# esrice/trio_binning

Hardware: AMD Instinct MI355X
Metric: Gbases/sec classified (k=21, 2x300M k-mer tables) (higher is better)
Workload: dtype u64

## Files before the change

trio_binning_amd/csrc/tbk_count.cpp:

```cpp
#include <hip/hip_runtime.h>

#include <algorithm>
#include <atomic>
#include <cerrno>
#include <cstdarg>
#include <cstdio>
#include <cstdlib>
#include <cstring>
#include <fcntl.h>
#include <string>
#include <thread>
#include <unistd.h>
#include <vector>

#include "../../include/tbk.h"
#include "tbk_common.h"
#include "tbk_compact_host.h"

extern "C" void tbk_set_error_(int code, const char *msg);
extern "C" hipError_t tbk_launch_separate(const uint8_t *, const uint64_t *, uint64_t, uint8_t *, hipStream_t);
extern "C" hipError_t tbk_launch_count(const uint8_t *, uint64_t, uint64_t, uint64_t, int, uint64_t *, uint32_t, TbkMz, int *, unsigned long long *,
                                       hipStream_t);
extern "C" uint64_t tbk_probe_passes(uint64_t total);
extern "C" hipError_t tbk_launch_count_clamp(uint64_t *, uint32_t, TbkMz, hipStream_t);
extern "C" hipError_t tbk_launch_count_rehash(uint64_t *, uint32_t, TbkMz, uint64_t *, uint32_t, TbkMz, int *, hipStream_t);
extern "C" hipError_t tbk_launch_count_histogram(uint64_t *, uint32_t, TbkMz, unsigned long long *, hipStream_t);
extern "C" hipError_t tbk_launch_count_unique(uint64_t *, uint32_t, TbkMz, uint64_t *, uint32_t, TbkMz, int, uint32_t, uint32_t,
                                              uint64_t *, uint64_t, unsigned long long *, hipStream_t);
extern "C" hipError_t tbk_launch_sort_u64(const uint64_t *, uint64_t *, uint64_t, int, hipStream_t);
extern "C" hipError_t tbk_launch_retain(const uint8_t *, uint64_t, uint64_t *, uint64_t, hipStream_t);
extern "C" hipError_t tbk_launch_count_class(const uint64_t *, uint64_t, uint64_t, uint64_t, int, uint64_t *, uint32_t, TbkMz, int *, unsigned long long *,
                                             uint32_t, uint32_t, hipStream_t);
extern "C" hipError_t tbk_launch_count_distil(uint64_t *, uint32_t, TbkMz, uint32_t, uint64_t *, uint8_t *, uint64_t, unsigned long long *, hipStream_t);
extern "C" hipError_t tbk_launch_db_solid_keys(const uint64_t *, const uint8_t *, uint64_t, uint64_t *, uint64_t, unsigned long long *, hipStream_t);
extern "C" hipError_t tbk_launch_db_unique(const uint64_t *, const uint8_t *, uint64_t, const uint64_t *, uint64_t, int, uint32_t, uint32_t, uint64_t *,
                                           uint64_t, unsigned long long *, hipStream_t);

static int cfail(int code, const char *fmt, ...) {
    char buf[512];
    va_list ap;
    va_start(ap, fmt);
    vsnprintf(buf, sizeof buf, fmt, ap);
    va_end(ap);
    tbk_set_error_(code, buf);
    return code;
}
#define CHIP(expr)                                                                                                      \
    do {                                                                                                                \
        hipError_t e_ = (expr);                                                                                         \
        if (e_ != hipSuccess)                                                                                           \
            return cfail(e_ == hipErrorOutOfMemory ? TBK_ERR_NOMEM : TBK_ERR_HIP, "%s: %s", #expr, hipGetErrorString(e_)); \
    } while (0)

struct tbk_counter {
    int device = 0, k = 0;
    uint64_t *d_lines = nullptr;
    uint32_t n_buckets = 0;
    TbkMz mz{0, 0, 0, 0};
    int *d_failed = nullptr;
    unsigned long long *d_used = nullptr;
    uint64_t since_clamp = 0;
    uint64_t used = 0;
    double load = 0.6;
    uint8_t *d_raw = nullptr, *d_sep = nullptr;
    uint64_t *d_off = nullptr;
    size_t cap_raw = 0, cap_sep = 0, cap_reads = 0;
    uint64_t bases_added = 0, reads_added = 0;
    hipEvent_t ev0 = nullptr, ev1 = nullptr;
    uint64_t timed_launches = 0, timed_windows = 0;
    double timed_ms = 0.0;
    uint64_t peak_table_bytes = 0;
    bool finished = false;
    bool broken = false;
    int passes = 1;
    uint64_t store_limit = 0;
    struct Segment { uint64_t *d = nullptr; uint64_t cap = 0, used = 0; };
    struct Piece { uint32_t segment; uint64_t first, words; };
    std::vector<Segment> segments;
    std::vector<Piece> pieces;
    uint64_t store_bytes = 0, store_words = 0;
    struct ClassDb { uint64_t *d_keys = nullptr; uint8_t *d_counts = nullptr; uint64_t n = 0; };
    std::vector<ClassDb> db;
    uint64_t database_bytes = 0;
    unsigned long long *d_hist = nullptr;
    uint64_t hist[256] = {0};
    uint64_t distinct_done = 0;
    bool compress = false;
    tbk_hpc *hpc = nullptr;
    bool keep_singletons = false;
    uint32_t floor() const { return keep_singletons ? 1u : 2u; }
};

static int counter_device(const tbk_counter *c) {
    int n = 0;
    if (hipGetDeviceCount(&n) != hipSuccess || n <= 0) return cfail(TBK_ERR_NO_DEVICE, "no HIP device visible; libtbk_hip has no CPU fallback");
    CHIP(hipSetDevice(c->device));
    return TBK_OK;
}

static int alloc_lines(int k, uint64_t capacity, double load, uint64_t **d_lines, uint32_t *n_buckets, TbkMz *mz, uint64_t *peak) {
    uint64_t nb = (uint64_t)((double)capacity / (TBK_SLOTS_PER_BUCKET * load)) + 16;
    if (nb > 0x7FFFFFF0ull) return cfail(TBK_ERR_NOMEM, "%llu distinct k-mers are more than one table holds", (unsigned long long)capacity);
    const size_t bytes = (size_t)nb * 128;
    hipError_t e = hipMalloc((void **)d_lines, bytes);
    if (e == hipSuccess) e = hipMemset2D(*d_lines, 128, 0xFF, 64, nb);
    if (e == hipSuccess) e = hipMemset2D((uint8_t *)*d_lines + 64, 128, 0, 64, nb);
    if (e != hipSuccess) {
        if (*d_lines) (void)hipFree(*d_lines);
        *d_lines = nullptr;
        (void)hipGetLastError();
        return cfail(e == hipErrorOutOfMemory ? TBK_ERR_NOMEM : TBK_ERR_HIP, "counting table for %llu k-mers (%zu bytes): %s",
                     (unsigned long long)capacity, bytes, hipGetErrorString(e));
    }
    *n_buckets = (uint32_t)nb;
    if (peak && bytes > *peak) *peak = bytes;
    const char *ew = getenv("TBK_COUNT_W"), *em = getenv("TBK_COUNT_M");
    *mz = tbk_mz_params(k, ew ? atoi(ew) : 6, capacity, em ? atoi(em) : 0, 0);
    return TBK_OK;
}
// ... 31 lines not shown
    c->device = device; c->k = k;
    c->passes = o.passes; c->store_limit = o.store_limit_bytes;
    c->compress = o.compress != 0;
    c->keep_singletons = o.keep_singletons != 0;
    if (c->compress) {
        const int made = tbk_hpc_create(device, &c->hpc);
        if (made) { delete c; return made; }
    }
    if (c->passes > 1) capacity_kmers = std::max<uint64_t>(1, capacity_kmers / (uint64_t)c->passes);
    const char *ev = getenv("TBK_COUNT_LOAD");
    c->load = ev ? atof(ev) : 0.6;
    if (c->load < 0.05) c->load = 0.05;
    if (c->load > 0.9) c->load = 0.9;
    rc = alloc_lines(k, capacity_kmers, c->load, &c->d_lines, &c->n_buckets, &c->mz, &c->peak_table_bytes);
    hipError_t e = hipSuccess;
    if (!rc && c->passes > 1) {
        e = hipMalloc((void **)&c->d_hist, 256 * sizeof(unsigned long long));
        if (e == hipSuccess) e = hipMemset(c->d_hist, 0, 256 * sizeof(unsigned long long));
    }
    if (!rc) e = hipMalloc((void **)&c->d_failed, sizeof(int));
    if (!rc && e == hipSuccess) e = hipMalloc((void **)&c->d_used, 1025 * sizeof(unsigned long long));
    if (!rc && e == hipSuccess) e = hipMemset(c->d_failed, 0, sizeof(int));
    if (!rc && e == hipSuccess) e = hipMemset(c->d_used, 0, 1025 * sizeof(unsigned long long));
    if (!rc && e != hipSuccess) rc = cfail(TBK_ERR_HIP, "tbk_counter_create: %s", hipGetErrorString(e));
    if (rc) { tbk_counter_destroy(c); return rc; }
    *out = c;
    return TBK_OK;
}

static int counter_grow(tbk_counter *c, uint64_t capacity) {
    uint64_t *d_new = nullptr;
    uint32_t nb = 0;
    TbkMz mz{0, 0, 0, 0};
    int rc = alloc_lines(c->k, capacity, c->load, &d_new, &nb, &mz, &c->peak_table_bytes);
    if (rc) return rc;
    hipError_t e = tbk_launch_count_rehash(c->d_lines, c->n_buckets, c->mz, d_new, nb, mz, c->d_failed, nullptr);
    int failed = 0;
    if (e == hipSuccess) e = hipMemcpy(&failed, c->d_failed, sizeof failed, hipMemcpyDeviceToHost);
    if (e != hipSuccess || failed) {
        (void)hipFree(d_new);
        return cfail(TBK_ERR_HIP, "counting table rebuild failed: %s", e != hipSuccess ? hipGetErrorString(e) : "new table full");
    }
    (void)hipFree(c->d_lines);
    c->d_lines = d_new; c->n_buckets = nb; c->mz = mz;
    return TBK_OK;
}

extern "C" void tbk_counter_destroy(tbk_counter *c) {
    if (!c) return;
    if (hipSetDevice(c->device) == hipSuccess) {
        (void)hipDeviceSynchronize();
        if (c->ev0) (void)hipEventDestroy(c->ev0);
        if (c->ev1) (void)hipEventDestroy(c->ev1);
        for (void *p : {(void *)c->d_lines, (void *)c->d_failed, (void *)c->d_used, (void *)c->d_raw, (void *)c->d_sep, (void *)c->d_off, (void *)c->d_hist})
            if (p) (void)hipFree(p);
        for (const tbk_counter::Segment &s : c->segments)
            if (s.d) (void)hipFree(s.d);
        for (const tbk_counter::ClassDb &d : c->db) {
            if (d.d_keys) (void)hipFree(d.d_keys);
            if (d.d_counts) (void)hipFree(d.d_counts);
        }
    }
    tbk_hpc_destroy(c->hpc);
    delete c;
}

static int count_stream(tbk_counter *c, const void *d_stream, uint64_t sep_total, int cls) {
    const uint64_t passes = tbk_probe_passes(sep_total);
    for (uint64_t p0 = 0; p0 < passes;) {
        uint64_t slots = (uint64_t)c->n_buckets * TBK_SLOTS_PER_BUCKET;
        constexpr uint64_t piece_cap = 1u << 19;
        static_assert(piece_cap <= TBK_COUNT_GRID_BLOCKS, "a piece of count_stream must fit the grid of one tbk_count_kernel launch");
        const uint64_t piece = std::min<uint64_t>(std::max<uint64_t>(32768, slots / 4 / 2048), piece_cap);
        const uint64_t np = std::min(piece, passes - p0), windows = np * 2048;
        if ((double)(c->used + windows) > 0.85 * (double)slots) {
            uint64_t want = (uint64_t)((double)slots * c->load) * 2;
            while ((double)(c->used + windows) > 0.85 * ((double)want / c->load)) want *= 2;
            const int rc = counter_grow(c, want);
            if (rc) return rc;
            slots = (uint64_t)c->n_buckets * TBK_SLOTS_PER_BUCKET;
        }
        if (c->since_clamp + windows >= ((uint64_t)1 << 31)) {
            CHIP(tbk_launch_count_clamp(c->d_lines, c->n_buckets, c->mz, nullptr));
            c->since_clamp = 0;
        }
        c->since_clamp += windows;
        if (!c->ev0) { CHIP(hipEventCreate(&c->ev0)); CHIP(hipEventCreate(&c->ev1)); }
        CHIP(hipEventRecord(c->ev0, nullptr));
        if (cls < 0)
            CHIP(tbk_launch_count((const uint8_t *)d_stream, sep_total, p0, np, c->k, c->d_lines, c->n_buckets, c->mz, c->d_failed, c->d_used, nullptr));
        else
            CHIP(tbk_launch_count_class((const uint64_t *)d_stream, sep_total / 16, p0, np, c->k, c->d_lines, c->n_buckets, c->mz, c->d_failed, c->d_used,
                                        (uint32_t)c->passes, (uint32_t)cls, nullptr));
        CHIP(hipEventRecord(c->ev1, nullptr));
        int failed = 0;
        unsigned long long used = 0;
        CHIP(hipMemcpy(&failed, c->d_failed, sizeof failed, hipMemcpyDeviceToHost));
        {
            float ms = 0;
            CHIP(hipEventElapsedTime(&ms, c->ev0, c->ev1));
            c->timed_ms += ms; c->timed_launches++; c->timed_windows += std::min<uint64_t>(windows, sep_total - p0 * 2048);
        }
        CHIP(hipMemcpy(&used, c->d_used, sizeof used, hipMemcpyDeviceToHost));
        c->used = used;
        if (failed) return cfail(TBK_ERR_NOMEM, "counting table is full (%llu slots, %llu taken)", (unsigned long long)slots, used);
        p0 += np;
    }
    return TBK_OK;
}

static int store_append(tbk_counter *c, uint64_t sep_total, uint64_t **d_words, uint64_t *n_words) {
    const uint64_t words = (sep_total + 15) / 16;
    if (c->store_limit && (c->store_words + words) * 8 > c->store_limit)
        return cfail(TBK_ERR_NOMEM, "the retained store would pass its limit of %llu bytes: %llu bases are retained in %llu bytes, the next batch needs %llu more",
                     (unsigned long long)c->store_limit, (unsigned long long)c->bases_added, (unsigned long long)(c->store_words * 8),
                     (unsigned long long)(words * 8));
    if (c->segments.empty() || c->segments.back().cap - c->segments.back().used < words) {
        uint64_t cap = std::max<uint64_t>(words, std::max<uint64_t>((uint64_t)1 << 17, c->store_words / 2));
        if (c->store_limit) cap = std::max<uint64_t>(words, std::min<uint64_t>(cap, c->store_limit / 8 - c->store_words));
        tbk_counter::Segment seg;
        const hipError_t e = hipMalloc((void **)&seg.d, cap * 8);
        if (e != hipSuccess) {
            (void)hipGetLastError();
            return cfail(e == hipErrorOutOfMemory ? TBK_ERR_NOMEM : TBK_ERR_HIP, "the retained store cannot grow by %llu bytes (%s): %llu bases are retained in %llu bytes",
                         (unsigned long long)(cap * 8), hipGetErrorString(e), (unsigned long long)c->bases_added, (unsigned long long)c->store_bytes);
        }
        seg.cap = cap;
        c->segments.push_back(seg);
        c->store_bytes += cap * 8;
    }
    tbk_counter::Segment &seg = c->segments.back();
    CHIP(tbk_launch_retain(c->d_sep, sep_total, seg.d + seg.used, words, nullptr));
    c->pieces.push_back({(uint32_t)(c->segments.size() - 1), seg.used, words});
    *d_words = seg.d + seg.used;
    *n_words = words;
    seg.used += words;
    c->store_words += words;
    return TBK_OK;
}

static int distil_class(tbk_counter *c) {
    CHIP(tbk_launch_count_histogram(c->d_lines, c->n_buckets, c->mz, c->d_hist, nullptr));
    unsigned long long h[256];
    CHIP(hipMemcpy(h, c->d_hist, sizeof h, hipMemcpyDeviceToHost));
    uint64_t keep = 0;
    for (int i = (int)c->floor(); i < 256; i++) keep += h[i] - c->hist[i];
    c->distinct_done += h[0] - c->hist[0];
    for (int i = 0; i < 256; i++) c->hist[i] = h[i];
    tbk_counter::ClassDb d;
    c->db.push_back(d);
    tbk_counter::ClassDb &db = c->db.back();
    if (keep) {
        CHIP(hipMalloc((void **)&db.d_keys, keep * sizeof(uint64_t)));
        CHIP(hipMalloc((void **)&db.d_counts, keep));
    }
    unsigned long long got = 0;
    CHIP(hipMemset(c->d_used, 0, sizeof got));
    CHIP(tbk_launch_count_distil(c->d_lines, c->n_buckets, c->mz, c->floor(), db.d_keys, db.d_counts, keep, c->d_used, nullptr));
    CHIP(hipMemcpy(&got, c->d_used, sizeof got, hipMemcpyDeviceToHost));
    CHIP(hipMemset(c->d_used, 0, sizeof got));
    if (got != keep) return cfail(TBK_ERR_HIP, "distilling a class: %llu k-mers to keep by the histogram, %llu in the table", (unsigned long long)keep, got);
    db.n = keep;
    c->database_bytes += keep * 9;
    c->used = 0;
    c->since_clamp = 0;
    return TBK_OK;
}

static int counter_finish(tbk_counter *c) {
    if (c->finished) return TBK_OK;
    if (c->broken) return cfail(TBK_ERR_INVALID, "the counter failed while it was being finished");
    if (c->passes == 1) { c->finished = true; return TBK_OK; }
    int rc = counter_device(c);
    if (rc) return rc;
    c->broken = true;
    rc = distil_class(c);
    for (int cls = 1; !rc && cls < c->passes; cls++) {
        for (size_t i = 0; !rc && i < c->pieces.size(); i++) {
            const tbk_counter::Piece &pc = c->pieces[i];
            rc = count_stream(c, c->segments[pc.segment].d + pc.first, pc.words * 16, cls);
        }
        if (!rc) rc = distil_class(c);
    }
    if (rc) return rc;
    for (tbk_counter::Segment &sg : c->segments) (void)hipFree(sg.d);
    c->segments.clear(); c->pieces.clear();
    c->store_bytes = 0; c->store_words = 0;
    for (void **p : {(void **)&c->d_lines, (void **)&c->d_raw, (void **)&c->d_sep, (void **)&c->d_off}) {
        if (*p) (void)hipFree(*p);
        *p = nullptr;
    }
    c->n_buckets = 0; c->cap_raw = 0; c->cap_sep = 0; c->cap_reads = 0;
    tbk_hpc_destroy(c->hpc);
    c->hpc = nullptr;
    c->broken = false;
    c->finished = true;
    return TBK_OK;
}

extern "C" int tbk_counter_finish(tbk_counter *c) {
    if (!c) return cfail(TBK_ERR_INVALID, "counter is NULL");
    return counter_finish(c);
}

static int counter_run(tbk_counter *c, const uint8_t *d_bases, const uint64_t *d_offsets, uint64_t n_reads, uint64_t total) {
    if (c->hpc) {
        void *d_cb = nullptr, *d_co = nullptr;
        const int rc = tbk_hpc_compress_device(c->hpc, d_bases, d_offsets, n_reads, total, 1, &d_cb, &d_co, &total);
        if (rc) return rc;
        d_bases = (const uint8_t *)d_cb;
        d_offsets = (const uint64_t *)d_co;
    }
    const size_t need_sep = (size_t)total + n_reads + 64;
    if (need_sep > c->cap_sep) {
        if (c->d_sep) CHIP(hipFree(c->d_sep));
        c->d_sep = nullptr; c->cap_sep = 0;
        CHIP(hipMalloc((void **)&c->d_sep, need_sep + need_sep / 8));
        c->cap_sep = need_sep + need_sep / 8;
    }
    CHIP(tbk_launch_separate(d_bases, d_offsets, n_reads, c->d_sep, nullptr));
    const uint64_t sep_total = total + n_reads;
    int rc;
    if (c->passes > 1) {
        uint64_t *d_words = nullptr, n_words = 0;
        rc = store_append(c, sep_total, &d_words, &n_words);
        if (!rc) rc = count_stream(c, d_words, n_words * 16, 0);
    } else {
        rc = count_stream(c, c->d_sep, sep_total, -1);
    }
    if (rc) return rc;
    c->bases_added += total;
    c->reads_added += n_reads;
    return TBK_OK;
}

extern "C" int tbk_check_offsets_(const uint64_t *offsets, uint64_t n_reads);

extern "C" int tbk_counter_add_batch(tbk_counter *c, const uint8_t *bases, const uint64_t *offsets, uint64_t n_reads) {
    if (!c || (n_reads && (!bases || !offsets))) return cfail(TBK_ERR_INVALID, "NULL argument");
    if (c->finished || c->broken) return cfail(TBK_ERR_INVALID, "the counter is finished: no more reads can be added");
    if (!n_reads) return TBK_OK;
    int rc = tbk_check_offsets_(offsets, n_reads);
    if (rc) return rc;
    rc = counter_device(c);
    if (rc) return rc;
    const uint64_t total = offsets[n_reads];
    if (total + 16 > c->cap_raw) {
        if (c->d_raw) CHIP(hipFree(c->d_raw));
        c->d_raw = nullptr; c->cap_raw = 0;
        CHIP(hipMalloc((void **)&c->d_raw, total + total / 8 + 64));
        c->cap_raw = total + total / 8 + 64;
    }
    if (n_reads + 1 > c->cap_reads) {
        if (c->d_off) CHIP(hipFree(c->d_off));
        c->d_off = nullptr; c->cap_reads = 0;
        CHIP(hipMalloc((void **)&c->d_off, (n_reads + n_reads / 8 + 2) * sizeof(uint64_t)));
        c->cap_reads = n_reads + n_reads / 8 + 2;
    }
    CHIP(hipMemcpy(c->d_raw, bases, total, hipMemcpyHostToDevice));
    CHIP(hipMemcpy(c->d_off, offsets, (n_reads + 1) * sizeof(uint64_t), hipMemcpyHostToDevice));
    return counter_run(c, c->d_raw, c->d_off, n_reads, total);
}

extern "C" int tbk_counter_add_device(tbk_counter *c, const void *d_bases, const void *d_offsets, uint64_t n_reads, uint64_t total_bases) {
    if (!c || (n_reads && (!d_bases || !d_offsets))) return cfail(TBK_ERR_INVALID, "NULL argument");
    if (c->finished || c->broken) return cfail(TBK_ERR_INVALID, "the counter is finished: no more reads can be added");
    if (!n_reads) return TBK_OK;
    int rc = counter_device(c);
    if (rc) return rc;
    return counter_run(c, (const uint8_t *)d_bases, (const uint64_t *)d_offsets, n_reads, total_bases);
}

extern "C" int tbk_counter_kernel_timing(tbk_counter *c, uint64_t *launches, uint64_t *window_starts, double *total_ms, int reset) {
    if (!c) return cfail(TBK_ERR_INVALID, "counter is NULL");
    if (launches) *launches = c->timed_launches;
    if (window_starts) *window_starts = c->timed_windows;
    if (total_ms) *total_ms = c->timed_ms;
    if (reset) { c->timed_launches = 0; c->timed_windows = 0; c->timed_ms = 0.0; }
    return TBK_OK;
}

// ... 1104 lines not shown
```

trio_binning_amd/csrc/tbk_count_kernels.hip:

```cpp
#include <hip/hip_runtime.h>
#include <rocprim/device/device_scan.hpp>
#include <stdint.h>

#include <type_traits>

#include "tbk_common.h"
#include "tbk_compact.h"
#include "tbk_device.h"


static uint32_t g_stream_blocks = 0, g_entry_blocks = 0;
extern "C" int tbk_count_set_grid_caps_(uint32_t stream_blocks, uint32_t entry_blocks) {
    g_stream_blocks = stream_blocks;
    g_entry_blocks = entry_blocks;
    return 0;
}
static inline unsigned stream_grid(uint64_t blocks) { return (unsigned)(g_stream_blocks && blocks > g_stream_blocks ? g_stream_blocks : blocks); }
static inline unsigned entry_grid(uint64_t blocks) { return (unsigned)(g_entry_blocks && blocks > g_entry_blocks ? g_entry_blocks : blocks); }

__global__ void __launch_bounds__(256)
tbk_separate_kernel(const uint8_t *__restrict__ bases, const uint64_t *__restrict__ offsets, uint64_t n_reads,
                    uint8_t *__restrict__ out) {
    const uint32_t lane = threadIdx.x & 63u;
    const uint64_t waves = (uint64_t)gridDim.x * (blockDim.x >> 6);
    for (uint64_t r = (uint64_t)blockIdx.x * (blockDim.x >> 6) + (threadIdx.x >> 6); r < n_reads; r += waves) {
        const uint64_t lo = offsets[r], hi = offsets[r + 1];
        uint8_t *dst = out + lo + r;
        for (uint64_t i = lo + lane; i < hi; i += 64) dst[i - lo] = bases[i] & 0xDFu;
        if (lane == 0) dst[hi - lo] = 'N';
    }
}

__global__ void __launch_bounds__(256)
tbk_retain_kernel(const uint8_t *__restrict__ sep, uint64_t total, uint64_t *__restrict__ store, uint64_t n_chunks) {
    for (uint64_t c = (uint64_t)blockIdx.x * blockDim.x + threadIdx.x; c < n_chunks; c += (uint64_t)gridDim.x * blockDim.x)
        store[c] = load_chunk(sep, c * 16, total);
}

struct TbkClassSel {
    uint32_t n_classes, cls;
};

constexpr int TBK_COUNT_LINE = 16;
struct TbkCountView {
    uint64_t *lines;
    uint32_t n_buckets;
    TbkMz mz;
    __device__ __forceinline__ unsigned long long *keys(uint32_t b) const { return (unsigned long long *)(lines + (uint64_t)b * TBK_COUNT_LINE); }
    __device__ __forceinline__ uint32_t *counts(uint32_t b) const { return (uint32_t *)(lines + (uint64_t)b * TBK_COUNT_LINE + TBK_SLOTS_PER_BUCKET); }
};

constexpr uint32_t TBK_COUNT_MAX_WALK = 1u << 12;

__device__ __forceinline__ bool count_from(const TbkCountView &t, uint64_t key, uint32_t b, bool at_home, uint32_t n, uint32_t &claimed) {
    for (uint32_t walked = 0; walked <= t.n_buckets && walked < TBK_COUNT_MAX_WALK; walked++) {
        unsigned long long *line = t.keys(b);
        for (int s = 0; s < TBK_SLOTS_PER_BUCKET; s++) {
            unsigned long long cur = __hip_atomic_load(&line[s], __ATOMIC_RELAXED, __HIP_MEMORY_SCOPE_AGENT);
            if (cur == TBK_EMPTY) {
                cur = atomicCAS(&line[s], (unsigned long long)TBK_EMPTY, (unsigned long long)key);
                if (cur == TBK_EMPTY) { cur = key; claimed++; }
            }
            if (cur == key) { atomicAdd(&t.counts(b)[s], n); return true; }
        }
        b = tbk_next_bucket(key, t.mz, t.n_buckets, b, at_home && walked == 0);
    }
    return false;
}

template <int W, bool M64, typename... Sel>
__global__ void __launch_bounds__(64)
tbk_count_kernel(const uint8_t *__restrict__ bases, uint64_t total, uint64_t first_pass, uint64_t n_passes, int k, TbkCountView t,
                 int *__restrict__ failed, unsigned long long *__restrict__ used, Sel... sel) {
    static_assert(sizeof...(Sel) == 0 || (sizeof...(Sel) == 1 && (std::is_same<Sel, TbkClassSel>::value && ...)), "at most one class selector");
    constexpr bool PACKED = sizeof...(Sel) == 1;
    __shared__ uint64_t stage[TBK_CHUNKS + 2];
    const uint32_t lane = threadIdx.x & 63u;
    const uint64_t kmask = k == 32 ? ~0ull : ((1ull << (2 * k)) - 1ull);
    const uint32_t badk = k == 32 ? 0xFFFFFFFFu : ((1u << k) - 1u);
    using win_t = typename std::conditional<M64, uint64_t, uint32_t>::type;
    const int m = t.mz.m, o = t.mz.o;
    const uint64_t mmask = m >= 32 ? ~0ull : ((1ull << (2 * m)) - 1ull);
    auto mmer_order = [&](uint64_t fwd64, uint64_t rc64, uint32_t fsh, uint32_t bsh) -> win_t {
        if (M64) {
            const uint64_t x = (fwd64 >> fsh) & mmask, y = (rc64 >> bsh) & mmask;
            return (win_t)tbk_mmer_hash64(x < y ? x : y);
        }
        const uint32_t x = (uint32_t)(fwd64 >> fsh) & (uint32_t)mmask, y = (uint32_t)(rc64 >> bsh) & (uint32_t)mmask;
        return (win_t)tbk_mmer_hash(x < y ? x : y);
    };
    for (uint64_t pass = first_pass + blockIdx.x; pass < first_pass + n_passes; pass += gridDim.x) {
        const uint64_t P0 = pass * TBK_PASS;
        __builtin_amdgcn_fence(__ATOMIC_ACQ_REL, "wavefront");
        if constexpr (PACKED) {
            const uint64_t *store = reinterpret_cast<const uint64_t *>(bases);
            const uint64_t c0 = P0 / 16, n_chunks = total / 16;
            auto word = [&](uint64_t c) -> uint64_t { return c < n_chunks ? store[c] : 0xFFFFull << 32; };
            stage[lane] = word(c0 + lane);
            stage[64 + lane] = word(c0 + 64 + lane);
            if (lane < 2) stage[128 + lane] = word(c0 + 128 + lane);
        } else {
            stage[lane] = load_chunk(bases, P0 + (uint64_t)lane * 16, total);
            stage[64 + lane] = load_chunk(bases, P0 + (uint64_t)(64 + lane) * 16, total);
            if (lane < 2) stage[128 + lane] = load_chunk(bases, P0 + (uint64_t)(128 + lane) * 16, total);
        }
        __builtin_amdgcn_fence(__ATOMIC_ACQ_REL, "wavefront");
        const uint64_t e0 = stage[2 * lane], e1 = stage[2 * lane + 1], e2 = stage[2 * lane + 2], e3 = stage[2 * lane + 3];
        uint32_t s0 = (uint32_t)e0, s1 = (uint32_t)e1, s2 = (uint32_t)e2, s3 = (uint32_t)e3;
        const unsigned __int128 R128 = (unsigned __int128)rev_pairs(~s3) | ((unsigned __int128)rev_pairs(~s2) << 32) |
                                       ((unsigned __int128)rev_pairs(~s1) << 64) | ((unsigned __int128)rev_pairs(~s0) << 96);
        const unsigned __int128 Rs = R128 >> (64 - 2 * k);
        uint32_t t0 = (uint32_t)Rs, t1 = (uint32_t)(Rs >> 32), t2 = (uint32_t)(Rs >> 64), t3 = (uint32_t)(Rs >> 96);
        uint32_t bad_lo = (uint32_t)(e0 >> 32) | ((uint32_t)(e1 >> 32) << 16);
        uint32_t bad_hi = (uint32_t)(e2 >> 32) | ((uint32_t)(e3 >> 32) << 16);
        win_t win[W > 0 ? W : 1];
        uint32_t fsh_new = 0, bsh_new = 0;
        if (W > 0) {
            const uint64_t fs = ((uint64_t)s1 << 32) | s0, bs = ((uint64_t)t3 << 32) | t2;
            win[0] = (win_t)~0ull;
#pragma unroll
            for (int i = 0; i + 1 < W; i++) win[i + 1] = mmer_order(fs, bs, (uint32_t)(2 * (o + i)), (uint32_t)(2 * (o + W - 1 - i)));
            fsh_new = (uint32_t)(2 * (o + W - 1));
            bsh_new = (uint32_t)(2 * o);
        }
        uint64_t held[TBK_SLOTS_PER_BUCKET];
#pragma unroll
        for (int s = 0; s < TBK_SLOTS_PER_BUCKET; s++) held[s] = 0;
        uint32_t held_bk = 0xFFFFFFFFu;
        uint32_t claimed = 0;
        uint32_t adds = 0;
        bool full = false;
        uint32_t pend_bk = 0xFFFFFFFFu;
        unsigned long long pend[4] = {0, 0, 0, 0};
        auto flush = [&]() {
            if (pend_bk == 0xFFFFFFFFu) return;
            unsigned long long *words = reinterpret_cast<unsigned long long *>(t.counts(pend_bk));
#pragma unroll
            for (int w = 0; w < 4; w++)
                if (pend[w]) { atomicAdd(&words[w], pend[w]); pend[w] = 0; adds++; }
        };
#pragma unroll 2
        for (int j = 0; j < TBK_WPL; j++) {
            const uint64_t fwd = ((uint64_t)s0 | ((uint64_t)s1 << 32)) & kmask;
            const uint64_t rc = ((uint64_t)t2 | ((uint64_t)t3 << 32)) & kmask;
            const uint64_t key = fwd < rc ? fwd : rc;
            bool ok = (bad_lo & badk) == 0 && P0 + (uint64_t)lane * TBK_WPL + (uint64_t)j + (uint64_t)k <= total;
            if constexpr (PACKED) {
                const TbkClassSel cs = (sel, ...);
                ok = ok && tbk_class_of(key, cs.n_classes) == cs.cls;
            }
            uint32_t hsel;
            if (W > 0) {
#pragma unroll
                for (int i = 0; i + 1 < W; i++) win[i] = win[i + 1];
                win[W - 1] = mmer_order(((uint64_t)s1 << 32) | s0, ((uint64_t)t3 << 32) | t2, fsh_new, bsh_new);
                win_t best = win[0];
#pragma unroll
                for (int i = 1; i < W; i++) best = win[i] < best ? win[i] : best;
                hsel = M64 ? (uint32_t)best : tbk_scramble((uint32_t)best);
            } else {
                hsel = tbk_mix32(key);
            }
            if (ok) {
                uint32_t b = tbk_reduce(hsel, t.n_buckets);
                bool done = false;
                for (uint32_t walked = 0; !done && walked < TBK_COUNT_MAX_WALK; walked++) {
                    unsigned long long *line = t.keys(b);
                    if (b != held_bk) {
                        const ulonglong2 *v = reinterpret_cast<const ulonglong2 *>(line);
                        const ulonglong2 v0 = v[0], v1 = v[1], v2 = v[2], v3 = v[3];
                        held[0] = v0.x; held[1] = v0.y; held[2] = v1.x; held[3] = v1.y;
                        held[4] = v2.x; held[5] = v2.y; held[6] = v3.x; held[7] = v3.y;
                        held_bk = b;
                    }
#pragma unroll
                    for (int s = 0; s < TBK_SLOTS_PER_BUCKET; s++) {
                        if (done) continue;
                        if (held[s] == TBK_EMPTY) {
                            const unsigned long long old = atomicCAS(&line[s], (unsigned long long)TBK_EMPTY, (unsigned long long)key);
                            held[s] = old == TBK_EMPTY ? key : old;
                            claimed += old == TBK_EMPTY ? 1u : 0u;
                        }
                        if (held[s] == key) {
                            if (b != pend_bk) { flush(); pend_bk = b; }
                            pend[s >> 1] += 1ull << (32 * (s & 1));
                            done = true;
                        }
                    }
                    if (!done) b = tbk_next_bucket(key, t.mz, t.n_buckets, b, walked == 0);
                }
                if (!done) full = true;
            }
            s0 = (s0 >> 2) | (s1 << 30); s1 = (s1 >> 2) | (s2 << 30); s2 = (s2 >> 2) | (s3 << 30); s3 >>= 2;
            t3 = (t3 << 2) | (t2 >> 30); t2 = (t2 << 2) | (t1 >> 30); t1 = (t1 << 2) | (t0 >> 30); t0 <<= 2;
            bad_lo = (bad_lo >> 1) | (bad_hi << 31); bad_hi >>= 1;
        }
        flush();
        if (full) atomicExch(failed, 1);
        uint32_t sum = claimed;
        for (int d = 32; d > 0; d >>= 1) sum += __shfl_xor(sum, d);
// ... 397 lines not shown
                                  const uint64_t *__restrict__ a_keys, uint64_t n_a, const uint64_t *__restrict__ flags,
                                  const unsigned long long *__restrict__ tile_offsets, uint64_t *__restrict__ out_keys,
                                  uint8_t *__restrict__ out_counts, uint64_t n_out) {
    __shared__ uint64_t bound[2];
    const uint64_t first = (uint64_t)blockIdx.x * TBK_DBT_TILE;
    compact_tile_bounds(b_keys, n_b, first, a_keys, n_a, bound, 0);
    __syncthreads();
    const uint64_t a_lo = bound[0], a_hi = bound[1];
    for (uint32_t r = 0; r < TBK_DBT_TILE / 256; r++) {
        const uint64_t j = first + (uint64_t)r * 256 + threadIdx.x;
        if (j >= n_b) continue;
        const uint64_t key = b_keys[j];
        const uint64_t rank = db_lower_bound(a_keys, a_lo, a_hi, key);
        if (rank < n_a && a_keys[rank] == key) continue;
        const uint64_t a_tile = rank / TBK_DBT_TILE;
        const uint32_t in_tile = (uint32_t)(rank % TBK_DBT_TILE), whole = in_tile >> 6, bits = in_tile & 63u;
        uint64_t dups = tile_offsets[a_tile];
        for (uint32_t w = 0; w < whole; w++) dups += (uint64_t)__popcll(flags[a_tile * TBK_DBT_WORDS + w]);
        if (bits) dups += (uint64_t)__popcll(flags[a_tile * TBK_DBT_WORDS + whole] & ((1ull << bits) - 1ull));
        const uint64_t at = j + rank - dups;
        if (at < n_out) {
            out_keys[at] = key;
            out_counts[at] = b_counts[j];
        }
    }
}

__global__ void __launch_bounds__(256)
tbk_kmerdb_tally_kernel(const uint8_t *__restrict__ counts, uint64_t n, unsigned long long *__restrict__ hist) {
    __shared__ unsigned int h[256];
    h[threadIdx.x] = 0;
    __syncthreads();
    for (uint64_t i = (uint64_t)blockIdx.x * blockDim.x + threadIdx.x; i < n; i += (uint64_t)gridDim.x * blockDim.x) atomicAdd(&h[counts[i]], 1u);
    __syncthreads();
    if (h[threadIdx.x]) atomicAdd(&hist[threadIdx.x], (unsigned long long)h[threadIdx.x]);
}

extern "C" hipError_t tbk_launch_separate(const uint8_t *d_bases, const uint64_t *d_offsets, uint64_t n_reads, uint8_t *d_out,
                                          hipStream_t stream) {
    if (!n_reads) return hipSuccess;
    uint64_t blocks = (n_reads + 3) / 4;
    if (blocks > 262144) blocks = 262144;
    hipLaunchKernelGGL(tbk_separate_kernel, dim3(stream_grid(blocks)), dim3(256), 0, stream, d_bases, d_offsets, n_reads, d_out);
    return hipGetLastError();
}

extern "C" hipError_t tbk_launch_count_rehash(uint64_t *from_lines, uint32_t from_buckets, TbkMz from_mz, uint64_t *to_lines,
                                              uint32_t to_buckets, TbkMz to_mz, int *d_failed, hipStream_t stream) {
    hipLaunchKernelGGL(tbk_count_rehash_kernel, dim3(entry_grid(8192)), dim3(256), 0, stream, TbkCountView{from_lines, from_buckets, from_mz},
                       TbkCountView{to_lines, to_buckets, to_mz}, d_failed);
    return hipGetLastError();
}

extern "C" hipError_t tbk_launch_count(const uint8_t *d_sep, uint64_t total, uint64_t first_pass, uint64_t n_passes, int k,
                                       uint64_t *d_lines, uint32_t n_buckets, TbkMz mz, int *d_failed, unsigned long long *d_used,
                                       hipStream_t stream) {
    if (total < (uint64_t)k || !n_passes) return hipSuccess;
    const uint64_t blocks = stream_grid(n_passes < TBK_COUNT_GRID_BLOCKS ? n_passes : TBK_COUNT_GRID_BLOCKS);
    const TbkCountView view{d_lines, n_buckets, mz};
    const dim3 grid((unsigned)blocks), block(64);
    const bool m64 = mz.m > 16;
#define TBK_COUNT_LAUNCH(N) case N: if (m64) hipLaunchKernelGGL((tbk_count_kernel<N, true>), grid, block, 0, stream, d_sep, total, first_pass, n_passes, k, view, d_failed, d_used); \
                                    else hipLaunchKernelGGL((tbk_count_kernel<N, false>), grid, block, 0, stream, d_sep, total, first_pass, n_passes, k, view, d_failed, d_used); break;
    switch (mz.t > 0 ? -1 : mz.w) {
        case 0: hipLaunchKernelGGL((tbk_count_kernel<0, false>), grid, block, 0, stream, d_sep, total, first_pass, n_passes, k, view, d_failed, d_used); break;
        TBK_COUNT_LAUNCH(1) TBK_COUNT_LAUNCH(2) TBK_COUNT_LAUNCH(3) TBK_COUNT_LAUNCH(4)
        TBK_COUNT_LAUNCH(5) TBK_COUNT_LAUNCH(6) TBK_COUNT_LAUNCH(7) TBK_COUNT_LAUNCH(8)
        default: return hipErrorInvalidValue;
    }
#undef TBK_COUNT_LAUNCH
    return hipGetLastError();
}

extern "C" hipError_t tbk_launch_count_histogram(uint64_t *d_lines, uint32_t n_buckets, TbkMz mz, unsigned long long *d_hist,
                                                 hipStream_t stream) {
    hipLaunchKernelGGL(tbk_count_histogram_kernel, dim3(entry_grid(4096)), dim3(256), 0, stream, TbkCountView{d_lines, n_buckets, mz}, d_hist);
    return hipGetLastError();
}

extern "C" hipError_t tbk_launch_count_unique(uint64_t *a_lines, uint32_t a_buckets, TbkMz a_mz, uint64_t *b_lines, uint32_t b_buckets,
                                              TbkMz b_mz, int k, uint32_t ci, uint32_t cx, uint64_t *d_out, uint64_t capacity,
                                              unsigned long long *d_n, hipStream_t stream) {
    hipLaunchKernelGGL(tbk_count_unique_kernel, dim3(entry_grid(8192)), dim3(256), 0, stream, TbkCountView{a_lines, a_buckets, a_mz},
                       TbkCountView{b_lines, b_buckets, b_mz}, k, ci, cx, d_out, capacity, d_n);
    return hipGetLastError();
}

extern "C" hipError_t tbk_launch_retain(const uint8_t *d_sep, uint64_t total, uint64_t *d_store, uint64_t n_chunks, hipStream_t stream) {
    if (!n_chunks) return hipSuccess;
    const uint64_t blocks = (n_chunks + 255) / 256;
    hipLaunchKernelGGL(tbk_retain_kernel, dim3(stream_grid(blocks < 65536 ? blocks : 65536)), dim3(256), 0, stream, d_sep, total, d_store, n_chunks);
    return hipGetLastError();
}

extern "C" hipError_t tbk_launch_count_class(const uint64_t *d_store, uint64_t n_chunks, uint64_t first_pass, uint64_t n_passes, int k,
                                             uint64_t *d_lines, uint32_t n_buckets, TbkMz mz, int *d_failed, unsigned long long *d_used,
                                             uint32_t n_classes, uint32_t cls, hipStream_t stream) {
    const uint64_t total = n_chunks * 16;
    if (total < (uint64_t)k || !n_passes) return hipSuccess;
    if (!n_classes || cls >= n_classes) return hipErrorInvalidValue;
    const uint64_t blocks = stream_grid(n_passes < TBK_COUNT_GRID_BLOCKS ? n_passes : TBK_COUNT_GRID_BLOCKS);
    const TbkCountView view{d_lines, n_buckets, mz};
    const TbkClassSel sel{n_classes, cls};
    const uint8_t *d_bases = reinterpret_cast<const uint8_t *>(d_store);
    const dim3 grid((unsigned)blocks), block(64);
    const bool m64 = mz.m > 16;
#define TBK_COUNT_LAUNCH(N) case N: if (m64) hipLaunchKernelGGL((tbk_count_kernel<N, true, TbkClassSel>), grid, block, 0, stream, d_bases, total, first_pass, n_passes, k, view, d_failed, d_used, sel); \
                                    else hipLaunchKernelGGL((tbk_count_kernel<N, false, TbkClassSel>), grid, block, 0, stream, d_bases, total, first_pass, n_passes, k, view, d_failed, d_used, sel); break;
    switch (mz.t > 0 ? -1 : mz.w) {
        case 0: hipLaunchKernelGGL((tbk_count_kernel<0, false, TbkClassSel>), grid, block, 0, stream, d_bases, total, first_pass, n_passes, k, view, d_failed, d_used, sel); break;
        TBK_COUNT_LAUNCH(1) TBK_COUNT_LAUNCH(2) TBK_COUNT_LAUNCH(3) TBK_COUNT_LAUNCH(4)
        TBK_COUNT_LAUNCH(5) TBK_COUNT_LAUNCH(6) TBK_COUNT_LAUNCH(7) TBK_COUNT_LAUNCH(8)
        default: return hipErrorInvalidValue;
    }
#undef TBK_COUNT_LAUNCH
    return hipGetLastError();
}

extern "C" hipError_t tbk_launch_count_distil(uint64_t *d_lines, uint32_t n_buckets, TbkMz mz, uint32_t floor, uint64_t *d_keys, uint8_t *d_counts,
                                              uint64_t capacity, unsigned long long *d_n, hipStream_t stream) {
    if (floor < 1 || floor > 2) return hipErrorInvalidValue;
    hipLaunchKernelGGL(tbk_count_distil_kernel, dim3(entry_grid(4096)), dim3(256), 0, stream, TbkCountView{d_lines, n_buckets, mz}, floor, d_keys, d_counts, capacity, d_n);
    return hipGetLastError();
}

extern "C" hipError_t tbk_launch_db_unique(const uint64_t *a_keys, const uint8_t *a_counts, uint64_t n_a, const uint64_t *b_sorted, uint64_t n_b,
                                           int k, uint32_t ci, uint32_t cx, uint64_t *d_out, uint64_t capacity, unsigned long long *d_n,
                                           hipStream_t stream) {
    if (!n_a) return hipSuccess;
    const uint64_t blocks = (n_a + 255) / 256;
    hipLaunchKernelGGL(tbk_db_unique_kernel, dim3(entry_grid(blocks < 8192 ? blocks : 8192)), dim3(256), 0, stream, a_keys, a_counts, n_a, b_sorted, n_b,
                       k, ci, cx, d_out, capacity, d_n);
    return hipGetLastError();
}

extern "C" hipError_t tbk_launch_count_export(uint64_t *d_lines, uint32_t n_buckets, TbkMz mz, int k, uint32_t floor, uint64_t *d_keys, uint8_t *d_counts,
                                              uint64_t capacity, unsigned long long *d_n, hipStream_t stream) {
    if (floor < 1 || floor > 2) return hipErrorInvalidValue;
    hipLaunchKernelGGL(tbk_count_export_kernel, dim3(entry_grid(4096)), dim3(256), 0, stream, TbkCountView{d_lines, n_buckets, mz}, k, floor, d_keys, d_counts, capacity, d_n);
    return hipGetLastError();
}

extern "C" hipError_t tbk_launch_db_rank(const uint64_t *d_keys, const uint8_t *d_counts, uint64_t n, int k, uint64_t *d_out_keys,
                                         uint8_t *d_out_counts, hipStream_t stream) {
    if (!n) return hipSuccess;
    const uint64_t blocks = (n + 255) / 256;
    hipLaunchKernelGGL(tbk_db_rank_kernel, dim3(entry_grid(blocks < 8192 ? blocks : 8192)), dim3(256), 0, stream, d_keys, d_counts, n, k, d_out_keys, d_out_counts);
    return hipGetLastError();
}

extern "C" hipError_t tbk_launch_kmerdb_check(const uint64_t *d_keys, const uint8_t *d_counts, uint64_t n, int k, uint32_t floor,
                                              unsigned long long *d_tally, hipStream_t stream) {
    if (!n) return hipSuccess;
    if (floor < 1 || floor > 2) return hipErrorInvalidValue;
    const uint64_t high_mask = k >= 32 ? 0ull : ~0ull << (2 * k);
    const uint64_t blocks = (n + 255) / 256;
    hipLaunchKernelGGL(tbk_kmerdb_check_kernel, dim3(entry_grid(blocks < 1024 ? blocks : 1024)), dim3(256), 0, stream, d_keys, d_counts, n, high_mask, floor, d_tally);
    return hipGetLastError();
}

extern "C" hipError_t tbk_launch_kmerdb_unique(const uint64_t *a_keys, const uint8_t *a_counts, uint64_t n_a, const uint64_t *b_keys, uint64_t n_b,
                                               uint32_t ci, uint32_t cx, uint64_t *d_out, uint64_t capacity, unsigned long long *d_n,
                                               hipStream_t stream) {
// ... 91 lines not shown
```

Measured before the change: 224.3.

## Fuse read separation and packing into one tiled pack kernel feeding counting

Replaces the separate-then-retain pipeline (write an N-separated byte stream, then pack it into 16-base words) with a single tiled kernel. The kernel locates each tile's first read by galloping search over the offsets, stages the raw bases in shared memory, marks read ends with a bitmap and prefix scan, and writes packed words directly. The counting kernel now always consumes packed words instead of byte streams, removing one full intermediate buffer and its memory traffic. In exchange the pack kernel is more complex, relies on the offset search, and the per-k-mer end-of-stream bound check is dropped in favour of padding words.

```diff
diff --git a/trio_binning_amd/csrc/tbk_count.cpp b/trio_binning_amd/csrc/tbk_count.cpp
--- a/trio_binning_amd/csrc/tbk_count.cpp
+++ b/trio_binning_amd/csrc/tbk_count.cpp
@@ -19,7 +19,8 @@
 
 extern "C" void tbk_set_error_(int code, const char *msg);
 extern "C" hipError_t tbk_launch_separate(const uint8_t *, const uint64_t *, uint64_t, uint8_t *, hipStream_t);
-extern "C" hipError_t tbk_launch_count(const uint8_t *, uint64_t, uint64_t, uint64_t, int, uint64_t *, uint32_t, TbkMz, int *, unsigned long long *,
+extern "C" hipError_t tbk_launch_pack_reads(const uint8_t *, const uint64_t *, uint64_t, uint64_t, uint64_t *, hipStream_t);
+extern "C" hipError_t tbk_launch_count(const uint64_t *, uint64_t, uint64_t, uint64_t, int, uint64_t *, uint32_t, TbkMz, int *, unsigned long long *,
                                        hipStream_t);
 extern "C" uint64_t tbk_probe_passes(uint64_t total);
 extern "C" hipError_t tbk_launch_count_clamp(uint64_t *, uint32_t, TbkMz, hipStream_t);
@@ -28,7 +29,6 @@
 extern "C" hipError_t tbk_launch_count_unique(uint64_t *, uint32_t, TbkMz, uint64_t *, uint32_t, TbkMz, int, uint32_t, uint32_t,
                                               uint64_t *, uint64_t, unsigned long long *, hipStream_t);
 extern "C" hipError_t tbk_launch_sort_u64(const uint64_t *, uint64_t *, uint64_t, int, hipStream_t);
-extern "C" hipError_t tbk_launch_retain(const uint8_t *, uint64_t, uint64_t *, uint64_t, hipStream_t);
 extern "C" hipError_t tbk_launch_count_class(const uint64_t *, uint64_t, uint64_t, uint64_t, int, uint64_t *, uint32_t, TbkMz, int *, unsigned long long *,
                                              uint32_t, uint32_t, hipStream_t);
 extern "C" hipError_t tbk_launch_count_distil(uint64_t *, uint32_t, TbkMz, uint32_t, uint64_t *, uint8_t *, uint64_t, unsigned long long *, hipStream_t);
@@ -62,9 +62,9 @@
     uint64_t since_clamp = 0;
     uint64_t used = 0;
     double load = 0.6;
-    uint8_t *d_raw = nullptr, *d_sep = nullptr;
-    uint64_t *d_off = nullptr;
-    size_t cap_raw = 0, cap_sep = 0, cap_reads = 0;
+    uint8_t *d_raw = nullptr;
+    uint64_t *d_off = nullptr, *d_words = nullptr;
+    size_t cap_raw = 0, cap_words = 0, cap_reads = 0;
     uint64_t bases_added = 0, reads_added = 0;
     hipEvent_t ev0 = nullptr, ev1 = nullptr;
     uint64_t timed_launches = 0, timed_windows = 0;
@@ -202,7 +202,7 @@
         (void)hipDeviceSynchronize();
         if (c->ev0) (void)hipEventDestroy(c->ev0);
         if (c->ev1) (void)hipEventDestroy(c->ev1);
-        for (void *p : {(void *)c->d_lines, (void *)c->d_failed, (void *)c->d_used, (void *)c->d_raw, (void *)c->d_sep, (void *)c->d_off, (void *)c->d_hist})
+        for (void *p : {(void *)c->d_lines, (void *)c->d_failed, (void *)c->d_used, (void *)c->d_raw, (void *)c->d_words, (void *)c->d_off, (void *)c->d_hist})
             if (p) (void)hipFree(p);
         for (const tbk_counter::Segment &s : c->segments)
             if (s.d) (void)hipFree(s.d);
@@ -215,8 +215,8 @@
     delete c;
 }
 
-static int count_stream(tbk_counter *c, const void *d_stream, uint64_t sep_total, int cls) {
-    const uint64_t passes = tbk_probe_passes(sep_total);
+static int count_stream(tbk_counter *c, const uint64_t *d_words, uint64_t sep_total, int cls) {
+    const uint64_t passes = tbk_probe_passes(sep_total), n_words = (sep_total + 15) / 16;
     for (uint64_t p0 = 0; p0 < passes;) {
         uint64_t slots = (uint64_t)c->n_buckets * TBK_SLOTS_PER_BUCKET;
         constexpr uint64_t piece_cap = 1u << 19;
@@ -238,9 +238,9 @@
         if (!c->ev0) { CHIP(hipEventCreate(&c->ev0)); CHIP(hipEventCreate(&c->ev1)); }
         CHIP(hipEventRecord(c->ev0, nullptr));
         if (cls < 0)
-            CHIP(tbk_launch_count((const uint8_t *)d_stream, sep_total, p0, np, c->k, c->d_lines, c->n_buckets, c->mz, c->d_failed, c->d_used, nullptr));
+            CHIP(tbk_launch_count(d_words, n_words, p0, np, c->k, c->d_lines, c->n_buckets, c->mz, c->d_failed, c->d_used, nullptr));
         else
-            CHIP(tbk_launch_count_class((const uint64_t *)d_stream, sep_total / 16, p0, np, c->k, c->d_lines, c->n_buckets, c->mz, c->d_failed, c->d_used,
+            CHIP(tbk_launch_count_class(d_words, n_words, p0, np, c->k, c->d_lines, c->n_buckets, c->mz, c->d_failed, c->d_used,
                                         (uint32_t)c->passes, (uint32_t)cls, nullptr));
         CHIP(hipEventRecord(c->ev1, nullptr));
         int failed = 0;
@@ -259,8 +259,9 @@
     return TBK_OK;
 }
 
-static int store_append(tbk_counter *c, uint64_t sep_total, uint64_t **d_words, uint64_t *n_words) {
-    const uint64_t words = (sep_total + 15) / 16;
+static int store_append(tbk_counter *c, const uint8_t *d_bases, const uint64_t *d_offsets, uint64_t n_reads, uint64_t total, uint64_t **d_words,
+                        uint64_t *n_words) {
+    const uint64_t words = (total + n_reads + 15) / 16;
     if (c->store_limit && (c->store_words + words) * 8 > c->store_limit)
         return cfail(TBK_ERR_NOMEM, "the retained store would pass its limit of %llu bytes: %llu bases are retained in %llu bytes, the next batch needs %llu more",
                      (unsigned long long)c->store_limit, (unsigned long long)c->bases_added, (unsigned long long)(c->store_words * 8),
@@ -280,7 +281,7 @@
         c->store_bytes += cap * 8;
     }
     tbk_counter::Segment &seg = c->segments.back();
-    CHIP(tbk_launch_retain(c->d_sep, sep_total, seg.d + seg.used, words, nullptr));
+    CHIP(tbk_launch_pack_reads(d_bases, d_offsets, n_reads, total, seg.d + seg.used, nullptr));
     c->pieces.push_back({(uint32_t)(c->segments.size() - 1), seg.used, words});
     *d_words = seg.d + seg.used;
     *n_words = words;
@@ -336,11 +337,11 @@
     for (tbk_counter::Segment &sg : c->segments) (void)hipFree(sg.d);
     c->segments.clear(); c->pieces.clear();
     c->store_bytes = 0; c->store_words = 0;
-    for (void **p : {(void **)&c->d_lines, (void **)&c->d_raw, (void **)&c->d_sep, (void **)&c->d_off}) {
+    for (void **p : {(void **)&c->d_lines, (void **)&c->d_raw, (void **)&c->d_words, (void **)&c->d_off}) {
         if (*p) (void)hipFree(*p);
         *p = nullptr;
     }
-    c->n_buckets = 0; c->cap_raw = 0; c->cap_sep = 0; c->cap_reads = 0;
+    c->n_buckets = 0; c->cap_raw = 0; c->cap_words = 0; c->cap_reads = 0;
     tbk_hpc_destroy(c->hpc);
     c->hpc = nullptr;
     c->broken = false;
@@ -361,22 +362,22 @@
         d_bases = (const uint8_t *)d_cb;
         d_offsets = (const uint64_t *)d_co;
     }
-    const size_t need_sep = (size_t)total + n_reads + 64;
-    if (need_sep > c->cap_sep) {
-        if (c->d_sep) CHIP(hipFree(c->d_sep));
-        c->d_sep = nullptr; c->cap_sep = 0;
-        CHIP(hipMalloc((void **)&c->d_sep, need_sep + need_sep / 8));
-        c->cap_sep = need_sep + need_sep / 8;
-    }
-    CHIP(tbk_launch_separate(d_bases, d_offsets, n_reads, c->d_sep, nullptr));
     const uint64_t sep_total = total + n_reads;
     int rc;
     if (c->passes > 1) {
         uint64_t *d_words = nullptr, n_words = 0;
-        rc = store_append(c, sep_total, &d_words, &n_words);
+        rc = store_append(c, d_bases, d_offsets, n_reads, total, &d_words, &n_words);
         if (!rc) rc = count_stream(c, d_words, n_words * 16, 0);
     } else {
-        rc = count_stream(c, c->d_sep, sep_total, -1);
+        const size_t need = (size_t)((sep_total + 15) / 16);
+        if (need > c->cap_words) {
+            if (c->d_words) CHIP(hipFree(c->d_words));
+            c->d_words = nullptr; c->cap_words = 0;
+            CHIP(hipMalloc((void **)&c->d_words, (need + need / 8) * sizeof(uint64_t)));
+            c->cap_words = need + need / 8;
+        }
+        CHIP(tbk_launch_pack_reads(d_bases, d_offsets, n_reads, total, c->d_words, nullptr));
+        rc = count_stream(c, c->d_words, sep_total, -1);
     }
     if (rc) return rc;
     c->bases_added += total;
diff --git a/trio_binning_amd/csrc/tbk_count_kernels.hip b/trio_binning_amd/csrc/tbk_count_kernels.hip
--- a/trio_binning_amd/csrc/tbk_count_kernels.hip
+++ b/trio_binning_amd/csrc/tbk_count_kernels.hip
@@ -31,10 +31,104 @@
     }
 }
 
-__global__ void __launch_bounds__(256)
-tbk_retain_kernel(const uint8_t *__restrict__ sep, uint64_t total, uint64_t *__restrict__ store, uint64_t n_chunks) {
-    for (uint64_t c = (uint64_t)blockIdx.x * blockDim.x + threadIdx.x; c < n_chunks; c += (uint64_t)gridDim.x * blockDim.x)
-        store[c] = load_chunk(sep, c * 16, total);
+constexpr int TBK_PACK_THREADS = 128;
+constexpr int TBK_PACK_TILE = 32 * TBK_PACK_THREADS;
+constexpr int TBK_PACK_WORDS = TBK_PACK_TILE / 16 / TBK_PACK_THREADS;
+constexpr uint32_t TBK_PACK_MAX_BLOCKS = 1u << 20;
+
+__global__ void __launch_bounds__(TBK_PACK_THREADS)
+tbk_pack_reads_kernel(const uint8_t *__restrict__ bases, const uint64_t *__restrict__ offsets, uint64_t n_reads, uint64_t total,
+                      uint64_t *__restrict__ words, uint64_t n_words) {
+    __shared__ uint4 raw4[TBK_PACK_TILE / 16 + 2];
+    __shared__ uint32_t closing[TBK_PACK_THREADS];
+    __shared__ uint32_t before[TBK_PACK_THREADS];
+    __shared__ uint32_t wave_sum[TBK_PACK_THREADS / 64];
+    const uint32_t *raw32 = reinterpret_cast<const uint32_t *>(raw4);
+    const uint8_t *raw8 = reinterpret_cast<const uint8_t *>(raw4);
+    const uint32_t tid = threadIdx.x, lane = tid & 63u;
+    const uint64_t tile_words = TBK_PACK_TILE / 16;
+    const uint64_t n_tiles = (n_words + tile_words - 1) / tile_words;
+    for (uint64_t tile = blockIdx.x; tile < n_tiles; tile += gridDim.x) {
+        const uint64_t S0 = tile * TBK_PACK_TILE;
+        closing[tid] = 0;
+        uint64_t r0 = 0, above = n_reads;
+        {
+            uint64_t guess = (uint64_t)((double)S0 / (double)(total + n_reads) * (double)n_reads);
+            if (guess >= n_reads) guess = n_reads - 1;
+            uint64_t step = 1;
+            if (offsets[guess] + guess <= S0) {
+                r0 = guess;
+                while (r0 + step < n_reads && offsets[r0 + step] + r0 + step <= S0) { r0 += step; step *= 2; }
+                if (r0 + step < n_reads) above = r0 + step;
+            } else {
+                above = guess;
+                while (above > step && offsets[above - step] + above - step > S0) { above -= step; step *= 2; }
+                if (above > step) r0 = above - step;
+            }
+        }
+        while (above - r0 > 1) {
+            const uint64_t mid = r0 + (above - r0) / 2;
+            if (offsets[mid] + mid <= S0) r0 = mid; else above = mid;
+        }
+        const uint64_t raw_lo = S0 - r0;
+        const uint64_t raw_n = raw_lo >= total ? 0 : total - raw_lo < (uint64_t)TBK_PACK_TILE ? total - raw_lo : (uint64_t)TBK_PACK_TILE;
+        const uintptr_t first = reinterpret_cast<uintptr_t>(bases + raw_lo);
+        const uint32_t mis = (uint32_t)(first & 15u);
+        const uint32_t n_gran = raw_n ? (uint32_t)((mis + raw_n + 15) / 16) : 0u;
+        const uint4 *src = reinterpret_cast<const uint4 *>(first - mis);
+        for (uint32_t g = tid; g < n_gran; g += TBK_PACK_THREADS) raw4[g] = src[g];
+        __syncthreads();
+        for (uint64_t r = r0 + tid;; r += TBK_PACK_THREADS) {
+            bool in = false;
+            if (r < n_reads) {
+                const uint64_t e = offsets[r + 1] + r - S0;
+                in = e < (uint64_t)TBK_PACK_TILE;
+                if (in) atomicOr(&closing[e >> 5], 1u << (e & 31u));
+            }
+            if (!__syncthreads_and(in)) break;
+        }
+        const uint32_t mine = __popc(closing[tid]);
+        uint32_t upto = mine;
+        for (uint32_t d = 1; d < 64; d <<= 1) {
+            const uint32_t v = __shfl_up(upto, d);
+            if (lane >= d) upto += v;
+        }
+        if (lane == 63) wave_sum[tid >> 6] = upto;
+        __syncthreads();
+        for (uint32_t w = 0; w < (tid >> 6); w++) upto += wave_sum[w];
+        before[tid] = upto - mine;
+        __syncthreads();
+        const uint64_t n_left = n_reads - r0;
+#pragma unroll
+        for (uint32_t i = 0; i < (uint32_t)TBK_PACK_WORDS; i++) {
+            const uint32_t q = (i * TBK_PACK_THREADS + tid) * 16;
+            const uint32_t bits32 = closing[q >> 5], sh = q & 31u;
+            const uint32_t ends = (bits32 >> sh) & 0xFFFFu;
+            uint32_t j = before[q >> 5] + __popc(bits32 & ((1u << sh) - 1u));
+            uint32_t w[4] = {0, 0, 0, 0};
+            if (!ends && j < n_left) {
+                const uint32_t o = mis + q - j;
+                const uint32_t *d = raw32 + (o >> 2);
+                const uint32_t s8 = (o & 3u) * 8u;
+                const uint32_t a0 = d[0], a1 = d[1], a2 = d[2], a3 = d[3], a4 = d[4];
+                w[0] = __funnelshift_r(a0, a1, s8); w[1] = __funnelshift_r(a1, a2, s8);
+                w[2] = __funnelshift_r(a2, a3, s8); w[3] = __funnelshift_r(a3, a4, s8);
+            } else {
+#pragma unroll
+                for (uint32_t x = 0; x < 16; x++) {
+                    uint32_t b = 0;
+                    if (j < n_left) {
+                        if ((ends >> x) & 1u) { b = 'N'; j++; }
+                        else b = raw8[mis + q + x - j];
+                    }
+                    w[x >> 2] |= b << (8 * (x & 3));
+                }
+            }
+            const uint64_t c = tile * tile_words + i * TBK_PACK_THREADS + tid;
+            if (c < n_words) words[c] = pack16(make_uint4(w[0] & 0xDFDFDFDFu, w[1] & 0xDFDFDFDFu, w[2] & 0xDFDFDFDFu, w[3] & 0xDFDFDFDFu));
+        }
+        __syncthreads();
+    }
 }
 
 struct TbkClassSel {
@@ -70,10 +164,10 @@
 
 template <int W, bool M64, typename... Sel>
 __global__ void __launch_bounds__(64)
-tbk_count_kernel(const uint8_t *__restrict__ bases, uint64_t total, uint64_t first_pass, uint64_t n_passes, int k, TbkCountView t,
+tbk_count_kernel(const uint64_t *__restrict__ store, uint64_t total, uint64_t first_pass, uint64_t n_passes, int k, TbkCountView t,
                  int *__restrict__ failed, unsigned long long *__restrict__ used, Sel... sel) {
     static_assert(sizeof...(Sel) == 0 || (sizeof...(Sel) == 1 && (std::is_same<Sel, TbkClassSel>::value && ...)), "at most one class selector");
-    constexpr bool PACKED = sizeof...(Sel) == 1;
+    constexpr bool SELECTS = sizeof...(Sel) == 1;
     __shared__ uint64_t stage[TBK_CHUNKS + 2];
     const uint32_t lane = threadIdx.x & 63u;
     const uint64_t kmask = k == 32 ? ~0ull : ((1ull << (2 * k)) - 1ull);
@@ -92,17 +186,12 @@
     for (uint64_t pass = first_pass + blockIdx.x; pass < first_pass + n_passes; pass += gridDim.x) {
         const uint64_t P0 = pass * TBK_PASS;
         __builtin_amdgcn_fence(__ATOMIC_ACQ_REL, "wavefront");
-        if constexpr (PACKED) {
-            const uint64_t *store = reinterpret_cast<const uint64_t *>(bases);
+        {
             const uint64_t c0 = P0 / 16, n_chunks = total / 16;
             auto word = [&](uint64_t c) -> uint64_t { return c < n_chunks ? store[c] : 0xFFFFull << 32; };
             stage[lane] = word(c0 + lane);
             stage[64 + lane] = word(c0 + 64 + lane);
             if (lane < 2) stage[128 + lane] = word(c0 + 128 + lane);
-        } else {
-            stage[lane] = load_chunk(bases, P0 + (uint64_t)lane * 16, total);
-            stage[64 + lane] = load_chunk(bases, P0 + (uint64_t)(64 + lane) * 16, total);
-            if (lane < 2) stage[128 + lane] = load_chunk(bases, P0 + (uint64_t)(128 + lane) * 16, total);
         }
         __builtin_amdgcn_fence(__ATOMIC_ACQ_REL, "wavefront");
         const uint64_t e0 = stage[2 * lane], e1 = stage[2 * lane + 1], e2 = stage[2 * lane + 2], e3 = stage[2 * lane + 3];
@@ -144,8 +233,8 @@
             const uint64_t fwd = ((uint64_t)s0 | ((uint64_t)s1 << 32)) & kmask;
             const uint64_t rc = ((uint64_t)t2 | ((uint64_t)t3 << 32)) & kmask;
             const uint64_t key = fwd < rc ? fwd : rc;
-            bool ok = (bad_lo & badk) == 0 && P0 + (uint64_t)lane * TBK_WPL + (uint64_t)j + (uint64_t)k <= total;
-            if constexpr (PACKED) {
+            bool ok = (bad_lo & badk) == 0;
+            if constexpr (SELECTS) {
                 const TbkClassSel cs = (sel, ...);
                 ok = ok && tbk_class_of(key, cs.n_classes) == cs.cls;
             }
@@ -649,18 +738,37 @@
     return hipGetLastError();
 }
 
-extern "C" hipError_t tbk_launch_count(const uint8_t *d_sep, uint64_t total, uint64_t first_pass, uint64_t n_passes, int k,
+extern "C" hipError_t tbk_launch_pack_reads(const uint8_t *d_bases, const uint64_t *d_offsets, uint64_t n_reads, uint64_t total, uint64_t *d_words,
+                                            hipStream_t stream) {
+    if (!n_reads) return hipSuccess;
+    const uint64_t n_words = (total + n_reads + 15) / 16;
+    const uint64_t tiles = (n_words * 16 + TBK_PACK_TILE - 1) / TBK_PACK_TILE;
+    hipLaunchKernelGGL(tbk_pack_reads_kernel, dim3(stream_grid(tiles < TBK_PACK_MAX_BLOCKS ? tiles : TBK_PACK_MAX_BLOCKS)), dim3(TBK_PACK_THREADS), 0, stream,
+                       d_bases, d_offsets, n_reads, total, d_words, n_words);
+    return hipGetLastError();
+}
+
+extern "C" int tbk_count_pack_tile_(void) { return TBK_PACK_TILE; }
+extern "C" int tbk_count_pack_reads_(int dev, const void *d_bases, const void *d_offsets, uint64_t n_reads, uint64_t total, void *d_words) {
+    hipError_t e = hipSetDevice(dev);
+    if (e == hipSuccess) e = tbk_launch_pack_reads((const uint8_t *)d_bases, (const uint64_t *)d_offsets, n_reads, total, (uint64_t *)d_words, nullptr);
+    if (e == hipSuccess) e = hipDeviceSynchronize();
+    return (int)e;
+}
+
+extern "C" hipError_t tbk_launch_count(const uint64_t *d_words, uint64_t n_chunks, uint64_t first_pass, uint64_t n_passes, int k,
                                        uint64_t *d_lines, uint32_t n_buckets, TbkMz mz, int *d_failed, unsigned long long *d_used,
                                        hipStream_t stream) {
+    const uint64_t total = n_chunks * 16;
     if (total < (uint64_t)k || !n_passes) return hipSuccess;
     const uint64_t blocks = stream_grid(n_passes < TBK_COUNT_GRID_BLOCKS ? n_passes : TBK_COUNT_GRID_BLOCKS);
     const TbkCountView view{d_lines, n_buckets, mz};
     const dim3 grid((unsigned)blocks), block(64);
     const bool m64 = mz.m > 16;
-#define TBK_COUNT_LAUNCH(N) case N: if (m64) hipLaunchKernelGGL((tbk_count_kernel<N, true>), grid, block, 0, stream, d_sep, total, first_pass, n_passes, k, view, d_failed, d_used); \
-                                    else hipLaunchKernelGGL((tbk_count_kernel<N, false>), grid, block, 0, stream, d_sep, total, first_pass, n_passes, k, view, d_failed, d_used); break;
+#define TBK_COUNT_LAUNCH(N) case N: if (m64) hipLaunchKernelGGL((tbk_count_kernel<N, true>), grid, block, 0, stream, d_words, total, first_pass, n_passes, k, view, d_failed, d_used); \
+                                    else hipLaunchKernelGGL((tbk_count_kernel<N, false>), grid, block, 0, stream, d_words, total, first_pass, n_passes, k, view, d_failed, d_used); break;
     switch (mz.t > 0 ? -1 : mz.w) {
-        case 0: hipLaunchKernelGGL((tbk_count_kernel<0, false>), grid, block, 0, stream, d_sep, total, first_pass, n_passes, k, view, d_failed, d_used); break;
+        case 0: hipLaunchKernelGGL((tbk_count_kernel<0, false>), grid, block, 0, stream, d_words, total, first_pass, n_passes, k, view, d_failed, d_used); break;
         TBK_COUNT_LAUNCH(1) TBK_COUNT_LAUNCH(2) TBK_COUNT_LAUNCH(3) TBK_COUNT_LAUNCH(4)
         TBK_COUNT_LAUNCH(5) TBK_COUNT_LAUNCH(6) TBK_COUNT_LAUNCH(7) TBK_COUNT_LAUNCH(8)
         default: return hipErrorInvalidValue;
@@ -680,13 +788,6 @@
                                               unsigned long long *d_n, hipStream_t stream) {
     hipLaunchKernelGGL(tbk_count_unique_kernel, dim3(entry_grid(8192)), dim3(256), 0, stream, TbkCountView{a_lines, a_buckets, a_mz},
                        TbkCountView{b_lines, b_buckets, b_mz}, k, ci, cx, d_out, capacity, d_n);
-    return hipGetLastError();
-}
-
-extern "C" hipError_t tbk_launch_retain(const uint8_t *d_sep, uint64_t total, uint64_t *d_store, uint64_t n_chunks, hipStream_t stream) {
-    if (!n_chunks) return hipSuccess;
-    const uint64_t blocks = (n_chunks + 255) / 256;
-    hipLaunchKernelGGL(tbk_retain_kernel, dim3(stream_grid(blocks < 65536 ? blocks : 65536)), dim3(256), 0, stream, d_sep, total, d_store, n_chunks);
     return hipGetLastError();
 }
 
@@ -699,13 +800,12 @@
     const uint64_t blocks = stream_grid(n_passes < TBK_COUNT_GRID_BLOCKS ? n_passes : TBK_COUNT_GRID_BLOCKS);
     const TbkCountView view{d_lines, n_buckets, mz};
     const TbkClassSel sel{n_classes, cls};
-    const uint8_t *d_bases = reinterpret_cast<const uint8_t *>(d_store);
     const dim3 grid((unsigned)blocks), block(64);
     const bool m64 = mz.m > 16;
-#define TBK_COUNT_LAUNCH(N) case N: if (m64) hipLaunchKernelGGL((tbk_count_kernel<N, true, TbkClassSel>), grid, block, 0, stream, d_bases, total, first_pass, n_passes, k, view, d_failed, d_used, sel); \
-                                    else hipLaunchKernelGGL((tbk_count_kernel<N, false, TbkClassSel>), grid, block, 0, stream, d_bases, total, first_pass, n_passes, k, view, d_failed, d_used, sel); break;
+#define TBK_COUNT_LAUNCH(N) case N: if (m64) hipLaunchKernelGGL((tbk_count_kernel<N, true, TbkClassSel>), grid, block, 0, stream, d_store, total, first_pass, n_passes, k, view, d_failed, d_used, sel); \
+                                    else hipLaunchKernelGGL((tbk_count_kernel<N, false, TbkClassSel>), grid, block, 0, stream, d_store, total, first_pass, n_passes, k, view, d_failed, d_used, sel); break;
     switch (mz.t > 0 ? -1 : mz.w) {
-        case 0: hipLaunchKernelGGL((tbk_count_kernel<0, false, TbkClassSel>), grid, block, 0, stream, d_bases, total, first_pass, n_passes, k, view, d_failed, d_used, sel); break;
+        case 0: hipLaunchKernelGGL((tbk_count_kernel<0, false, TbkClassSel>), grid, block, 0, stream, d_store, total, first_pass, n_passes, k, view, d_failed, d_used, sel); break;
         TBK_COUNT_LAUNCH(1) TBK_COUNT_LAUNCH(2) TBK_COUNT_LAUNCH(3) TBK_COUNT_LAUNCH(4)
         TBK_COUNT_LAUNCH(5) TBK_COUNT_LAUNCH(6) TBK_COUNT_LAUNCH(7) TBK_COUNT_LAUNCH(8)
         default: return hipErrorInvalidValue;
```

After: 220.4. 0.983x the previous value.
